# 011235813/discrete_mean_field_game

Measured on AMD Instinct MI355X. Metric: env-steps/sec for batched d-bin population rollouts, higher is better.
Workload: dtype f32 (f64 accumulate); 1 GPU; actor_critic.train(update_every="rollout") of the drop-in class (mfg_ac2.train call surface; device-side start draw every episode, one update per 15-step rollout): d=21 topics, T=15, global batch 65536 = 65536 trajectories per GPU x 1; d=21, T=15, batch_per_gpu=65536, global_batch=65536, rng=philox4x32-10, parallelism=trajectory-sharded x1, 1 all-reduce/update

## Files before the change

discrete_mean_field_game_amd/csrc/mfg_core.h:

```cpp
#pragma once
#include <hip/hip_runtime.h>
#include <stdint.h>

#include <atomic>
#include <type_traits>

#include "../../include/mfg_hip.h"
#include "mfg_device.h"

namespace mfg {

constexpr int BLOCK = 256;
constexpr int WAVES = BLOCK / WAVE;

struct CoreArgs {
  const float* pi0;
  const int32_t* start_idx;
  int64_t num_start;
  int start_draw;
  const float* pi_alpha;
  union {
    const float* P_in;
    float* pi_start_out;
  };
// ... 175 lines not shown
  T al, ad, gt;
};
template <bool SAMPLE, bool FAST>
__device__ __forceinline__ PolicyTerms<FAST> policy_terms(const PolicyElem<FAST>& e, const float4* __restrict__ htab, float th,
                                                          float v) {
  PolicyTerms<FAST> o;
  if constexpr (FAST) {
#ifdef MFG_ABL_LNY
    const float lnv = v;
#else
    const float lnv = (!SAMPLE && v == 0.0f) ? (float)(LOG_ZERO_P * INV_LN2) : (SAMPLE ? __builtin_amdgcn_logf(v) : log2_pos(v));
#endif
    o.al = e.al_f;
    o.ad = e.ad_f;
    o.gt = __builtin_fmaf(lnv, e.ad_f, -e.psi_ad);
  } else {
    const double lnv = (!SAMPLE && v == 0.0f) ? LOG_ZERO_P : log((double)v);
    o.al = e.al_d;
    o.ad = e.ad_d;
    o.gt = (-digamma_pos(e.al_d) + lnv) * e.ad_d;
  }
  return o;
}

__device__ __forceinline__ float policy_term_denormal(const PolicyElem<true>& e, float v) {
  return __builtin_fmaf(log2_pos(v), e.ad_f, -e.psi_ad);
}

template <int NE, bool TD, bool FAST, bool SEP, bool ALLVALID = false>
__device__ __forceinline__ void sample_elems_gq(const CoreArgs& a, double theta, const ThetaSplit& ts, const float* pj,
                                                const float* ej, const float* pai, const float* Fi, const uint32_t* elem,
                                                const bool* valid, uint32_t qstep, uint32_t step, uint64_t traj, float* y,
                                                typename PolicyTerms<FAST>::T* al, typename PolicyTerms<FAST>::T* ad,
                                                typename PolicyTerms<FAST>::T* gt) {
  QuadRand q;
  quad_rand(q, a.seed, elem[0], qstep, traj);
#ifndef MFG_QUAD_WIDTH
#define MFG_QUAD_WIDTH 2
#endif
  constexpr int PW = MFG_QUAD_WIDTH;
#pragma unroll
  for (int h = 0; PW * h < NE; ++h) {
    const int n2 = (NE - PW * h) >= PW ? PW : (NE - PW * h);
    PolicyElem<FAST> pe[PW];
#pragma unroll
    for (int u = 0; u < PW; ++u) {
      if (u < n2) {
        const int e = PW * h + u;
        if constexpr (SEP) policy_setup_sep<true, TD>(pe[u], a, ts, pj[e], ej[e], pai[e], Fi[e]);
        else policy_setup<true, TD, FAST>(pe[u], a, theta, ts, pj[e], pai[e]);
      }
    }
    float xn[PW], v[PW];
    bool sure[PW];
#pragma unroll
    for (int u = 0; u < PW; u += 2) {
      const int hp = (PW * h + u) >> 1;
      sure[u] = true;
      if (u + 1 < PW) sure[u + 1] = true;
#ifdef MFG_ABL_BM
      xn[u] = (q.radu[hp] - 0.5f) * 2.0f;
      if (u + 1 < PW) xn[u + 1] = (q.radu[hp] - 0.5f) * q.ang[hp];
#else
      if (u < n2) {
        const float rad = __builtin_amdgcn_sqrtf(-__builtin_amdgcn_logf(q.radu[hp]));
        xn[u] = rad * __builtin_amdgcn_cosf(q.ang[hp]);
        if (u + 1 < PW) xn[u + 1] = rad * __builtin_amdgcn_sinf(q.ang[hp]);
      }
#endif
    }
    uint64_t coldm = 0;
#pragma unroll
    for (int u = 0; u < PW; ++u) {
      if (u < n2) {
        const int e = PW * h + u;
        uint64_t cm;
        if (quad_kbits(e) == 16) v[u] = gamma_try_mask<16>(pe[u].gs, xn[u], q.kf[e], cm);
        else v[u] = gamma_try_mask<12>(pe[u].gs, xn[u], q.kf[e], cm);
        y[e] = pe[u].gs.dd * v[u];
        if constexpr (ALLVALID) coldm |= cm;
        else coldm |= cm & __builtin_amdgcn_ballot_w64(valid[e]);
      }
    }
    const bool any_cold = coldm != 0;
    if (__builtin_expect(any_cold, 0)) {
#pragma unroll
      for (int u = 0; u < PW; ++u) {
        const int e = PW * h + u;
        if (u < n2 && (ALLVALID || valid[e])) {
          const bool k16 = quad_kbits(e) == 16;
          if (k16) (void)gamma_try<16>(pe[u].gs, xn[u], q.kf[e], sure[u]);
          else (void)gamma_try<12>(pe[u].gs, xn[u], q.kf[e], sure[u]);
          if (!sure[u] || pe[u].gs.small)
            y[e] = gamma_fix(pe[u].gs, xn[u], q.kf[e], k16 ? TryConst<16>::kscale : TryConst<12>::kscale, sure[u], v[u], a.seed,
                             elem[e], step, traj);
        }
      }
    }
#pragma unroll
    for (int u = 0; u < PW; ++u) {
      if (u < n2) {
        const int e = PW * h + u;
        if (TD) {
          const PolicyTerms<FAST> t = policy_terms<true, FAST>(pe[u], a.htab, ts.th, y[e]);
          al[e] = (ALLVALID || valid[e]) ? t.al : 0;
          ad[e] = (ALLVALID || valid[e]) ? t.ad : 0;
          gt[e] = (ALLVALID || valid[e]) ? t.gt : 0;
        }
        if (!ALLVALID && !valid[e]) y[e] = 0.0f;
      }
    }
    if constexpr (TD && FAST) {
      if (__builtin_expect(any_cold, 0)) {
#pragma unroll
        for (int u = 0; u < PW; ++u) {
          const int e = PW * h + u;
          if (u < n2 && (ALLVALID || valid[e]) && y[e] < FLT_MIN_NORMAL) gt[e] = policy_term_denormal(pe[u], y[e]);
        }
      }
    }
  }
}

template <int NE, bool TD, bool FAST, bool SEP>
__device__ __forceinline__ void sample_elems_g(const CoreArgs& a, double theta, const ThetaSplit& ts, const float* pj,
                                               const float* ej, const float* pai, const float* Fi, const uint32_t* elem,
                                               const bool* valid, uint32_t step, uint64_t traj, float* y,
                                               typename PolicyTerms<FAST>::T* al, typename PolicyTerms<FAST>::T* ad,
                                               typename PolicyTerms<FAST>::T* gt) {
  sample_elems_gq<NE, TD, FAST, SEP>(a, theta, ts, pj, ej, pai, Fi, elem, valid, step, step, traj, y, al, ad, gt);
}

template <int NE, bool TD, bool FAST, bool SEP>
__device__ __forceinline__ void sample_elems(const CoreArgs& a, double theta, const ThetaSplit& ts, const float* pj,
                                             const float* ej, float pai, float Fi, uint32_t elem0, uint32_t step,
                                             uint64_t traj, float* y, float& ys, typename PolicyTerms<FAST>::T& as,
                                             typename PolicyTerms<FAST>::T& ds, typename PolicyTerms<FAST>::T& gs) {
  using TT = typename PolicyTerms<FAST>::T;
  float pa[NE], fi[NE];
  uint32_t el[NE];
  bool ok[NE];
  TT al[NE], ad[NE], gt[NE];
#pragma unroll
  for (int e = 0; e < NE; ++e) {
    pa[e] = pai;
    fi[e] = Fi;
    el[e] = elem0 + (uint32_t)e;
    ok[e] = true;
  }
  sample_elems_g<NE, TD, FAST, SEP>(a, theta, ts, pj, ej, pa, fi, el, ok, step, traj, y, al, ad, gt);
  ys = y[0];
  if (TD) {
    as = al[0];
    ds = ad[0];
    gs = gt[0];
  }
#pragma unroll
  for (int e = 1; e < NE; ++e) {
    ys += y[e];
    if (TD) {
      as += al[e];
      ds += ad[e];
      gs += gt[e];
    }
  }
}

template <bool TD, bool FAST, bool SEP>
__device__ __forceinline__ void sample_tail1(const CoreArgs& a, double theta, const ThetaSplit& ts, float pj, float ej, float pai,
                                             float Fi, uint32_t elem, uint32_t step, uint64_t traj, bool& have, float& cxn,
                                             float& ckf, float& y, typename PolicyTerms<FAST>::T& al,
                                             typename PolicyTerms<FAST>::T& ad, typename PolicyTerms<FAST>::T& gt) {
  PolicyElem<FAST> pe;
  if constexpr (SEP) policy_setup_sep<true, TD>(pe, a, ts, pj, ej, pai, Fi);
  else policy_setup<true, TD, FAST>(pe, a, theta, ts, pj, pai);
  const bool odd = (step & 1u) != 0;
  float xn, kf;
  if (odd && have) {
    xn = cxn;
    kf = ckf;
    have = false;
  } else {
    QuadRand q;
// ... 9 lines not shown
  static_assert(quad_kbits(0) == 16 && quad_kbits(1) == 16, "both integers of the first pair are 16-bit");
  uint64_t cm;
  float v = gamma_try_mask<16>(pe.gs, xn, kf, cm);
  y = pe.gs.dd * v;
  if (__builtin_expect(cm != 0, 0)) {
    bool sure = true;
    (void)gamma_try<16>(pe.gs, xn, kf, sure);
    if (!sure || pe.gs.small) y = gamma_fix(pe.gs, xn, kf, TryConst<16>::kscale, sure, v, a.seed, elem, step, traj);
  }
  if (TD) {
    const PolicyTerms<FAST> t = policy_terms<true, FAST>(pe, a.htab, ts.th, y);
    al = t.al;
    ad = t.ad;
    gt = t.gt;
    if constexpr (FAST) {
      if (__builtin_expect(cm != 0, 0) && y < FLT_MIN_NORMAL) gt = policy_term_denormal(pe, y);
    }
  }
}

__device__ __forceinline__ double value_wave(const float* pis, const double* __restrict__ w, int d, int lane) {
  const int Q = d * (d + 1) / 2;
  double acc = 0.0;
  for (int c = lane; c < d; c += WAVE) {
    const double pc = (double)pis[c];
    double col = 0.0;
    for (int i = 0; i <= c; ++i) col = fma(w[feat_idx(i, c, d)], (double)pis[i], col);
    acc = fma(pc, col + w[Q + c], acc);
  }
  acc = wave_sum(acc);
  return acc + w[Q + d];
}

#ifndef MFG_CORE_SMALL_WAVES
#define MFG_CORE_SMALL_WAVES 3
#endif
template <bool SAMPLE, bool TD, bool FAST, int D, bool SUMS = false, int STEP = 0>
#ifndef MFG_CORE_SMALL_WAVES_F64
#define MFG_CORE_SMALL_WAVES_F64 3
#endif
__device__ __forceinline__ void core_small_body(const CoreArgs& a) {
  extern __shared__ __attribute__((aligned(16))) unsigned char smem_raw[];
  MFG_STAMP0(8)
  MFG_STAMPB(0)
  const int d = D ? D : a.d;
  const int dd = d * d, dp = d | 1, T = a.T;
  const int G = WAVE / d, TB = WAVES * G;
  const int Q = d * (d + 1) / 2, F = Q + d + 1;
  const bool want_v = TD && a.w != nullptr;
  constexpr bool CIRC = SAMPLE && D > 0 && (D & 1);
  constexpr int H = (D + 1) / 2;
  const int pnw = CIRC ? 2 * d : d;
  double* wl = reinterpret_cast<double*>(smem_raw);
  double* pis64 = wl + (want_v ? ((F + 1) & ~1) : 0);
  double* red = pis64 + (SAMPLE ? 2 * TB * d : 0);
  float* tile = reinterpret_cast<float*>(red + 4 * TB * d);
  float* pis = tile + TB * d * dp;
  float* pex = pis + TB * d;
  float* pin = pex + TB * d;
  float* pal = pin + TB * 2 * d;
  double* scal = reinterpret_cast<double*>(pal + TB * d + ((TB * d) & 1));
  double* tot = scal + TB * 3;
  float* pst = reinterpret_cast<float*>(tot + TB * 8);
  const int tid = threadIdx.x, lane = tid & (WAVE - 1), wv = tid / WAVE;
  const int t = lane / d, i = lane - t * d;
  auto nblk_f = [&]() -> unsigned { return STEP == 1 ? gridDim.x - (unsigned)core_step_red_blocks(F + 3) : gridDim.x; };
  if constexpr (STEP == 1) {
    if (blockIdx.x >= nblk_f()) {
      const int64_t k = (int64_t)(blockIdx.x - nblk_f()) * WAVES + wv;
      const int64_t FO = F + 3;
      if (k >= FO) return;
      double old_val = 0.0;
      if (lane == 0) {
        if (k < F) old_val = a.w_out[k];
        else if (k == F) old_val = *a.theta;
        else if (k == F + 1 && a.pend_reward_acc) old_val = *a.pend_reward_acc;
      }
      const double gk = rows_column_sum(a.step_rows, a.step_nrows, FO, k, lane);
      if (lane == 0) {
        const double inv = 1.0 / (double)a.B;
        a.step_G[k] = gk;
        if (k < F) a.w_out[k] = updated_param(old_val, a.pend_lr_c, gk, inv);
        else if (k == F) *a.theta_out = updated_param(old_val, a.pend_lr_a, gk, inv);
        else if (k == F + 1 && a.pend_reward_acc) *a.pend_reward_acc = old_val + gk * inv;
      }
      return;
    }
  }
  float pi_first = 0.0f;
  if constexpr (STEP == 1) {
    const int64_t b0f = (int64_t)blockIdx.x * TB;
    const int tlf = wv * G + t;
    if (b0f < a.B) {
      const int64_t bf = b0f + ((t < G && b0f + tlf < a.B) ? tlf : 0);
      pi_first = a.pi0[core_src_row(a, bf) * d + i];
    }
// ... 65 lines not shown
      if (H & 1) c0 = fma(wl[(H - 1) * d + i], (double)vec[i + H - 1], c0);
      col = c0 + c1;
    } else {
      for (int k = 0, idx = i; k <= i; idx += d - k - 1, ++k) col = fma(wl[idx], (double)vec[k], col);
    }
    return (double)pi_e * (col + wl[Q + i]);
  };
  const int64_t ntiles = (a.B + TB - 1) / TB;
  for (int64_t tileid = blockIdx.x; tileid < ntiles; tileid += nblk_f()) {
    const int64_t b0 = tileid * TB;
    const int nb = (int)((a.B - b0) < TB ? (a.B - b0) : TB);
    const int tl = wv * G + t;
    const bool valid = (t < G) && (tl < nb);
    const int tlc = valid ? tl : 0;
    const int64_t b = b0 + tlc;
    double* redq = red + (size_t)tlc * 4 * d;
    float* pnv = pin + tlc * pnw;
    float pi_i = pi_first;
    {
      const int64_t tn = tileid + nblk_f();
      if (tn < ntiles) {
        const int64_t b0n = tn * TB;
        const int64_t bn = b0n + ((t < G && b0n + tl < a.B) ? tl : 0);
        pi_first = a.pi0[core_src_row(a, bn) * d + i];
      }
    }
    if (valid && a.pi_traj) a.pi_traj[b * (int64_t)(T + 1) * d + i] = pi_i;
    if constexpr (STEP == 2) {
      if (valid && a.pi_start_out) a.pi_start_out[b * d + i] = pi_i;
    }
    double v_cur = 0.0, discount = 1.0;
    bool tail_have = false;
    float tail_xn = 0.0f, tail_kf = 0.0f;
    MFG_STAMP0(10)
    for (int s = 0; s < T; ++s) {
      MFG_STAMP(0)
      tile_sync();
      float Fi = 0.0f;
      if (valid) {
        pis[tlc * d + i] = pi_i;
        if (SAMPLE && want_v && s == 0) {
          pst[tlc * pnw + i] = pi_i;
          if (CIRC) pst[tlc * pnw + d + i] = pi_i;
        }
        if (SAMPLE) pis64[2 * (tlc * d + i)] = (double)pi_i;
        if (sep) {
          pex[tlc * d + i] = exp_f64arg(theta * ((double)pi_i - SEP_CENTRE));
          Fi = exp_f64arg(-theta * ((double)pi_i + (a.shift - SEP_CENTRE)));
        }
      }
      if (!SAMPLE) {
        const int n = nb * dd;
        const float* src = a.P_in + b0 * dd;
        for (int k = tid; k < n; k += BLOCK) {
          const int row = (int)(((float)k + 0.5f) * inv_d);
          const int colj = k - row * d;
          tile[row * dp + colj] = src[k];
        }
        if (a.pi_next_in)
          for (int k = tid; k < nb * d; k += BLOCK) pin[k] = a.pi_next_in[b0 * d + k];
        if (a.pi_alpha)
          for (int k = tid; k < nb * d; k += BLOCK) pal[k] = a.pi_alpha[b0 * d + k];
      }
      tile_sync();
      MFG_STAMP(1)
      float* trow = tile + (tlc * d + i) * dp;
      const float* pv = pis + tlc * d;
      const float* pav = (!SAMPLE && a.pi_alpha) ? pal + tlc * d : pv;
      const float pai = pav[i];
      const double pid = (double)pi_i;
      double A = 0.0, D_ = 0.0, Ssum = 0.0, gacc = 0.0, racc = 0.0;
      if (valid) {
        const uint32_t step = a.first_step + (uint32_t)s;
        const uint64_t traj = a.traj_offset + (uint64_t)b;
        if (SAMPLE) {
          using TT = typename PolicyTerms<FAST>::T;
          const float* ev = pex + tlc * d;
          const uint32_t erow = (uint32_t)(i * d);
          const float pas = sep ? pai + ts.sh : pai;
          const int dq = d & ~3;
          if constexpr (D > 0 && sep) {
            typedef __attribute__((address_space(3))) const float lds_cf;
            typedef __attribute__((address_space(3))) float lds_f;
            constexpr int EOFF = WAVES * (WAVE / D) * D;
            static_assert(EOFF + 3 <= 255, "E_j must sit inside the ds_read2_b32 offset field of the pi_j base");
            lds_cf* rp = (lds_cf*)pav;
            lds_f* wp = (lds_f*)trow;
            auto quad = [&](int j, float& ys, TT& as, TT& ds, TT& gs) __attribute__((always_inline)) {
              float y[4], pjv[4], ejv[4];
#pragma unroll
              for (int e = 0; e < 4; ++e) {
                pjv[e] = rp[e];
                ejv[e] = rp[EOFF + e];
              }
              sample_elems<4, TD, FAST, sep>(a, theta, ts, pjv, ejv, pas, Fi, erow + (uint32_t)j, step, traj, y, ys, as, ds, gs);
#pragma unroll
              for (int e = 0; e < 4; ++e) wp[e] = y[e];
              rp += 4;
              wp += 4;
              asm volatile("" : "+v"(rp), "+v"(wp));
            };
#ifndef MFG_QUAD_UNROLL
#define MFG_QUAD_UNROLL 1
#endif
#pragma unroll MFG_QUAD_UNROLL
            for (int j = 0; j < dq; j += 4) {
              float ys;
              TT as, ds, gs;
              quad(j, ys, as, ds, gs);
              Ssum += (double)ys;
              if (TD) {
                A += (double)as;
                D_ += (double)ds;
                gacc += (double)gs;
              }
            }
          } else
#pragma unroll 1
          for (int j = 0; j < dq; j += 4) {
            float y[4], ys = 0.0f;
            TT as = 0, ds = 0, gs = 0;
            sample_elems<4, TD, FAST, sep>(a, theta, ts, pav + j, ev + j, pas, Fi, erow + (uint32_t)j, step, traj, y, ys,
                                           as, ds, gs);
#pragma unroll
            for (int e = 0; e < 4; ++e) trow[j + e] = y[e];
            Ssum += (double)ys;
            if (TD) {
              A += (double)as;
              D_ += (double)ds;
              gacc += (double)gs;
            }
          }
          if (dq < d) {
            float y[4], ys = 0.0f;
            TT as = 0, ds = 0, gs = 0;
            const int rem = d - dq;
            if (rem == 1)
              sample_tail1<TD, FAST, sep>(a, theta, ts, pav[dq], ev[dq], pas, Fi, erow + (uint32_t)dq, step, traj, tail_have, tail_xn,
                                          tail_kf, y[0], as, ds, gs), ys = y[0];
            else if (rem == 2)
              sample_elems<2, TD, FAST, sep>(a, theta, ts, pav + dq, ev + dq, pas, Fi, erow + (uint32_t)dq, step, traj, y,
                                             ys, as, ds, gs);
            else
              sample_elems<3, TD, FAST, sep>(a, theta, ts, pav + dq, ev + dq, pas, Fi, erow + (uint32_t)dq, step, traj, y,
                                             ys, as, ds, gs);
            for (int e = 0; e < rem; ++e) trow[dq + e] = y[e];
            Ssum += (double)ys;
            if (TD) {
              A += (double)as;
              D_ += (double)ds;
              gacc += (double)gs;
            }
          }
        } else {
          PolicyElem<FAST> pe;
#pragma unroll 2
          for (int j = 0; j < d; ++j) {
            policy_setup<SAMPLE, TD, FAST>(pe, a, theta, ts, pav[j], pai);
            const float p = trow[j];
            policy_accumulate<SAMPLE, TD, FAST>(pe, a.htab, ts.th, p, A, D_, gacc);
            racc += reward_term(a.reward_kind, pid, (double)pv[j], (double)p);
          }
        }
        MFG_STAMP(2)
        if (TD && FAST) gacc *= LN2;
        if (SAMPLE) {
          float* inv_slot = reinterpret_cast<float*>(pis64 + 2 * (tlc * d + i) + 1);
          if (FAST) {
            const float inv32 = fast_rcp_f32_of_f64(Ssum);
            if (a.P_out) {
              for (int j = 0; j < d; ++j) trow[j] *= inv32;
              *inv_slot = 1.0f;
// ... 308 lines not shown
            int k = -1;
            if (gj < D) {
              if (gi <= gj) k = feat_idx(gi, gj, D);
            } else if (gj == D) {
              if (gi <= D) k = Qc + gi;
            } else if (gj == D + 1) {
              if (gi == D) k = Fc;
            } else if (gj == D + 2) {
              if (gi == D + 1) k = Fc + 1;
            } else if (gj == D + 3) {
              if (gi == D + 1) k = Fc + 2;
            }
            const double val = tt == 0 ? c0[v] : (tt == 1 ? c1[v] : c2[v]);
            if (k >= 0) rows[wv * FO + k] = val;
          }
        }
        __syncthreads();
        for (int k = tid; k < FO; k += BLOCK) {
          double tsum = rows[k];
#pragma unroll
          for (int q = 1; q < WAVES; ++q) tsum += rows[q * FO + k];
          a.part_rows[tileid * FO + k] = tsum;
        }
        __syncthreads();
      }
    }
    MFG_STAMP0(11)
    MFG_STAMPB(1)
  }
}
template <bool SAMPLE, bool TD, bool FAST, int D, bool SUMS = false, int STEP = 0>
__global__ __launch_bounds__(BLOCK, SUMS ? 2 : (FAST ? MFG_CORE_SMALL_WAVES : MFG_CORE_SMALL_WAVES_F64)) void k_core_small(CoreArgs a) { core_small_body<SAMPLE, TD, FAST, D, SUMS, STEP>(a); }

inline size_t core_small_lds(int d, bool want_v, bool sample) {
  const int G = WAVE / d, TB = WAVES * G, dp = d | 1;
  const size_t F = (size_t)d * (d + 1) / 2 + d + 1;
  const size_t fl = (size_t)TB * d * dp + 5 * (size_t)TB * d;
  return (want_v ? ((F + 1) & ~(size_t)1) * 8 : 0) + (sample ? (size_t)2 * TB * d * 8 : 0) + (size_t)4 * TB * d * 8 + (fl + (fl & 1)) * 4 +
         (size_t)TB * 3 * 8 + (size_t)TB * 8 * 8 + (size_t)TB * 2 * d * 4;
}

#ifndef MFG_CORE_LARGE_WAVES
#define MFG_CORE_LARGE_WAVES(R) (((R) <= 2 || (R) == 4) ? 3 : 2)
#endif
#ifndef MFG_CORE_LARGE_WAVES_MIXED_SAMPLING
#define MFG_CORE_LARGE_WAVES_MIXED_SAMPLING(R) ((R) <= 2 ? 4 : ((R) <= 7 ? 3 : 2))
#endif
__host__ __device__ constexpr int large_row_batch(int R, bool td) { return R <= 2 ? 8 : (R <= 4 ? (td ? 8 : 4) : 2); }
inline size_t core_large_lds(int d, bool sample, bool fast, bool td) {
  const int R = (d + WAVE - 1) / WAVE;
  if (sample && fast) return (size_t)WAVES * ((td ? 5 : 2) * d + large_row_batch(R, td) * WAVE * R) * 4;
  return (size_t)WAVES * 4 * d * 4 + (size_t)WAVES * 3 * d * 8;
}
template <int R>
__device__ __forceinline__ void stash_store(float* p, const float* y) {
  if constexpr (R % 4 == 0) {
#pragma unroll
    for (int m = 0; m < R; m += 4) *reinterpret_cast<float4*>(p + m) = make_float4(y[m], y[m + 1], y[m + 2], y[m + 3]);
  } else if constexpr (R % 2 == 0) {
#pragma unroll
    for (int m = 0; m < R; m += 2) *reinterpret_cast<float2*>(p + m) = make_float2(y[m], y[m + 1]);
  } else {
#pragma unroll
    for (int m = 0; m < R; ++m) p[m] = y[m];
  }
}
template <int R>
__device__ __forceinline__ void stash_load(float* y, const float* p) {
  if constexpr (R % 4 == 0) {
#pragma unroll
    for (int m = 0; m < R; m += 4) {
      const float4 v = *reinterpret_cast<const float4*>(p + m);
// ... 484 lines not shown
```

discrete_mean_field_game_amd/csrc/mfg_core_small.hip:

```cpp
#include "mfg_core.h"

namespace mfg {

template <bool SAMPLE, bool TD, bool FAST, int D, bool SUMS = false, int STEP = 0>
static void go(const CoreArgs& a, int num_cus, size_t lds, hipStream_t st) {
  const int grid = core_small_grid<k_core_small<SAMPLE, TD, FAST, D, SUMS, STEP>>(a, lds, num_cus);
  hipLaunchKernelGGL((k_core_small<SAMPLE, TD, FAST, D, SUMS, STEP>), dim3(grid + (STEP == 1 ? core_step_red_blocks(a.d * (a.d + 1) / 2 + a.d + 1 + 3) : 0)), dim3(BLOCK), lds, st, a);
}

template <int D>
static void dispatch(const CoreArgs& a, bool sample, bool td, bool fast, int num_cus, size_t lds, hipStream_t st) {
  if constexpr (D > 0) {
    if (sample && td && a.step_nrows > 0) {
      if (fast) go<true, true, true, D, false, 1>(a, num_cus, lds, st);
      else go<true, true, false, D, false, 1>(a, num_cus, lds, st);
      return;
    }
    if (sample && td && a.step_nrows < 0) {
      if (fast) go<true, true, true, D, false, 2>(a, num_cus, lds, st);
      else go<true, true, false, D, false, 2>(a, num_cus, lds, st);
      return;
    }
    if (sample && td && a.part_rows) {
      if (fast) go<true, true, true, D, true>(a, num_cus, lds, st);
      else go<true, true, false, D, true>(a, num_cus, lds, st);
      return;
    }
  }
  if (fast) {
    if (sample && td) go<true, true, true, D>(a, num_cus, lds, st);
    else if (sample) go<true, false, true, D>(a, num_cus, lds, st);
    else go<false, true, true, D>(a, num_cus, lds, st);
  } else {
    if (sample && td) go<true, true, false, D>(a, num_cus, lds, st);
    else if (sample) go<true, false, false, D>(a, num_cus, lds, st);
    else go<false, true, false, D>(a, num_cus, lds, st);
  }
}

int launch_core_small(const CoreArgs& a, bool sample, bool td, bool fast, int num_cus, hipStream_t st) {
  const int d = a.d;
  if (core_row3_wanted(a, sample, td, fast, num_cus)) return launch_core_row3(a, td, num_cus, st);
  const bool want_v = td && a.w != nullptr;
  const size_t lds = core_small_lds(d, want_v, sample);
  if (d == 21) dispatch<21>(a, sample, td, fast, num_cus, lds, st);
  else if (d == 15) dispatch<15>(a, sample, td, fast, num_cus, lds, st);
  else dispatch<0>(a, sample, td, fast, num_cus, lds, st);
  return MFG_OK;
}

}
```

discrete_mean_field_game_amd/csrc/mfg_device.h:

```cpp
#pragma once
#include <hip/hip_runtime.h>
#include <stdint.h>

namespace mfg {

constexpr int WAVE = 64;
typedef double v4d_t __attribute__((ext_vector_type(4)));
constexpr float ZERO_GAMMA_REPLACEMENT = 1e-20f;
constexpr double LOG_ZERO_P = -230.25850929940458;
constexpr double LN2 = 0.6931471805599453, INV_LN2 = 1.4426950408889634;

struct u32x4 {
  uint32_t x, y, z, w;
};

__host__ __device__ __forceinline__ uint32_t xor3(uint32_t a, uint32_t b, uint32_t c) {
#if defined(__HIP_DEVICE_COMPILE__) && defined(__has_builtin)
#if __has_builtin(__builtin_amdgcn_bitop3_b32)
  return __builtin_amdgcn_bitop3_b32(a, b, c, 0x96);
#else
  return a ^ b ^ c;
#endif
#else
  return a ^ b ^ c;
#endif
}

__host__ __device__ __forceinline__ u32x4 philox4x32_10(u32x4 c, uint32_t k0, uint32_t k1) {
  constexpr uint32_t M0 = 0xD2511F53u, M1 = 0xCD9E8D57u, W0 = 0x9E3779B9u, W1 = 0xBB67AE85u;
#pragma unroll
  for (int r = 0; r < 10; ++r) {
    const uint64_t p0 = (uint64_t)M0 * c.x;
    const uint64_t p1 = (uint64_t)M1 * c.z;
    u32x4 n;
    n.x = xor3((uint32_t)(p1 >> 32), c.y, k0);
    n.y = (uint32_t)p1;
    n.z = xor3((uint32_t)(p0 >> 32), c.w, k1);
    n.w = (uint32_t)p0;
    c = n;
    k0 += W0;
    k1 += W1;
  }
  return c;
}

__device__ __forceinline__ u32x4 philox_elem(uint64_t seed, uint32_t elem, uint32_t step, uint64_t traj,
                                             uint32_t block) {
  u32x4 c;
  c.x = elem;
  c.y = step;
  c.z = (uint32_t)traj;
  c.w = ((uint32_t)(traj >> 32) & 0xFFFFu) | (block << 16);
  return philox4x32_10(c, (uint32_t)seed, (uint32_t)(seed >> 32));
}

__device__ __forceinline__ float u01(uint32_t r) { return __builtin_fmaf((float)(r >> 8), 5.9604644775390625e-8f, 2.98023223876953125e-8f); }

__device__ __forceinline__ float fast_ln(float x) { return __builtin_amdgcn_logf(x) * 0.69314718055994531f; }
__device__ __forceinline__ float fast_exp(float x) { return __builtin_amdgcn_exp2f(x * 1.44269504088896341f); }

constexpr float BM_K = 1.1774100225154747f;
constexpr float BM_K2 = 1.3862943611198906f;
struct GammaState {
  float a, dd, c;
  bool small;
};

__device__ __forceinline__ void gamma_setup(GammaState& g, float a) {
  g.a = a;
  g.small = a < 1.0f;
  const float a1 = g.small ? a + 1.0f : a;
  g.dd = a1 - (1.0f / 3.0f);
  g.c = __builtin_amdgcn_rsqf(9.0f * g.dd);
}
__device__ __forceinline__ void gamma_setup_hot(GammaState& g, float a) {
  g.a = a;
  g.small = a < 1.0f;
  g.dd = a - (1.0f / 3.0f);
  g.c = __builtin_amdgcn_rsqf((9.0f / BM_K2) * g.dd);
}
__device__ __forceinline__ void gamma_setup_hot(GammaState& g, float alpha, float scale, float scale9k) {
  g.dd = __builtin_fmaf(alpha, scale, -(1.0f / 3.0f));
  g.small = g.dd < (2.0f / 3.0f);
  g.a = g.dd + (1.0f / 3.0f);
  g.c = __builtin_amdgcn_rsqf(__builtin_fmaf(alpha, scale9k, -3.0f / BM_K2));
}

__device__ __forceinline__ bool mt_accept(const GammaState& g, float x, float u, float& v) {
  const float t = g.c * x;
  const float eps = t * (3.0f + t * (3.0f + t));
  const float x2 = x * x;
  const float tp = 1.0f + t;
  v = t < -0.5f ? tp * tp * tp : 1.0f + eps;
  bool acc = u < 1.0f - 0.0331f * x2 * x2;
  if (!acc) {
    float lme;
    if (__builtin_fabsf(eps) < 0.125f) {
      const float e2 = eps * eps;
      lme = e2 * (-0.5f + eps * (1.0f / 3.0f + eps * (-0.25f + eps * (0.2f + eps * (-1.0f / 6.0f +
            eps * (1.0f / 7.0f + eps * (-0.125f)))))));
    } else {
      lme = fast_ln(v) - eps;
    }
    acc = fast_ln(u) < 0.5f * x2 + g.dd * lme;
  }
  return acc && (t > -1.0f);
}

__device__ __forceinline__ float box_muller_radius(uint32_t r) {
  return __builtin_amdgcn_sqrtf(-1.3862943611198906f * __builtin_amdgcn_logf(u01(r)));
}

struct QuadRand {
  float radu[2];
  float ang[2];
  float kf[4];
};
__host__ __device__ constexpr int quad_kbits(int e) { return e < 2 ? 16 : 12; }

__device__ __forceinline__ void quad_rand(QuadRand& q, uint64_t seed, uint32_t elem0, uint32_t step, uint64_t traj) {
#ifdef MFG_ABL_PHILOX
  u32x4 r;
  r.x = (elem0 + step) * 2654435761u ^ (uint32_t)traj;
  r.y = r.x * 2246822519u + 12345u;
  r.z = r.y ^ (r.x >> 7);
  r.w = r.z * 3266489917u;
#else
  const u32x4 r = philox_elem(seed, elem0, step, traj, 0);
#endif
  q.ang[0] = __builtin_fmaf((float)(r.z >> 16), 1.52587890625e-5f, 7.62939453125e-6f);
  q.ang[1] = __builtin_fmaf((float)(r.z & 0xFFFFu), 1.52587890625e-5f, 7.62939453125e-6f);
  q.radu[0] = __builtin_fmaf((float)(r.x >> 12), 9.5367431640625e-7f, 4.76837158203125e-7f);
  q.radu[1] = __builtin_fmaf((float)(r.y >> 12), 9.5367431640625e-7f, 4.76837158203125e-7f);
  q.kf[0] = (float)(r.w >> 16);
  q.kf[1] = (float)(r.w & 0xFFFFu);
  q.kf[2] = (float)(r.x & 0xFFFu);
  q.kf[3] = (float)(r.y & 0xFFFu);
}

__device__ __forceinline__ float gamma_exact_path(const GammaState& g, float x, float kf, float kscale, uint64_t seed,
                                                  uint32_t elem, uint32_t step, uint64_t traj) {
  float v = 1.0f;
  {
    const u32x4 r = philox_elem(seed, elem, step, traj, 1);
    const float u = (kf + u01(r.x)) * kscale;
    if (mt_accept(g, x, u, v)) return v;
  }
  for (uint32_t block = 2; block < 64; ++block) {
    const u32x4 r = philox_elem(seed, elem, step, traj, block);
    const float xn = box_muller_radius(r.x) * __builtin_amdgcn_cosf(u01(r.y));
    if (mt_accept(g, xn, u01(r.z), v)) return v;
  }
  return 1.0f;
}

template <int KB>
struct TryConst {
  static constexpr float slope = KB == 16 ? -12451.84f * 1.3862944f : -778.24f * 1.3862944f;
  static constexpr float top = KB == 16 ? 65532.7f : 4094.85f;
  static constexpr float kscale = KB == 16 ? 1.52587890625e-5f : 2.44140625e-4f;
};
template <int KB = 12>
__device__ __forceinline__ float gamma_try(const GammaState& g, float x, float kf, bool& sure) {
#ifdef MFG_ABL_TRY
  sure = true;
  return 1.0f + 3.0f * g.c * x;
#endif
  const float t = g.c * x;
  const float q = x * t;
  const float thr = __builtin_fmaf(q * q, TryConst<KB>::slope, TryConst<KB>::top);
// ... 159 lines not shown
struct ThetaSplit {
  float th, tl, sh, c0;
  float thn;
};
__device__ __forceinline__ ThetaSplit theta_split(double theta, double shift) {
  ThetaSplit t;
  t.th = (float)theta;
  t.tl = (float)(theta - (double)t.th);
  t.sh = (float)shift;
  t.c0 = t.th * (float)(shift - (double)t.sh);
  t.thn = t.th * 16.0f;
  return t;
}
__device__ __forceinline__ void theta_times_x(const ThetaSplit& t, float pj, float pi, float& x, float& zh, float& zl) {
  x = (pj - pi) - t.sh;
  zh = t.th * x;
  zl = __builtin_fmaf(t.th, x, -zh) + __builtin_fmaf(t.tl, x, -t.c0);
}

constexpr float HTAB_ZMIN = -24.0f;
constexpr float HTAB_ZMAX = 88.0f;
constexpr int HTAB_PER_UNIT = 16;
constexpr int HTAB_N = (88 + 24) * HTAB_PER_UNIT;

__device__ __forceinline__ float htab_eval(const float4* __restrict__ tab, float x, float thn) {
#ifdef MFG_ABL_HTAB
  return x * thn * 0.1f;
#endif
  static_assert(HTAB_PER_UNIT == 16, "ThetaSplit::thn assumes 16 intervals per unit of z");
  float t = __builtin_fmaf(x, thn, -HTAB_ZMIN * (float)HTAB_PER_UNIT);
  t = __builtin_amdgcn_fmed3f(t, 0.0f, (float)HTAB_N - 0.001f);
  const unsigned k = (unsigned)t;
  const float f = __builtin_amdgcn_fractf(t);
  const float4 c = tab[k];
  return __builtin_fmaf(__builtin_fmaf(__builtin_fmaf(c.w, f, c.z), f, c.y), f, c.x);
}

template <int CTRL, int ROW_MASK>
__device__ __forceinline__ double dpp_mov_f64(double v) {
  int lo = __double2loint(v), hi = __double2hiint(v);
  if (ROW_MASK == 0xF) {
    lo = __builtin_amdgcn_update_dpp(0, lo, CTRL, 0xF, 0xF, true);
    hi = __builtin_amdgcn_update_dpp(0, hi, CTRL, 0xF, 0xF, true);
  } else {
    lo = __builtin_amdgcn_update_dpp(0, lo, CTRL, ROW_MASK, 0xF, false);
    hi = __builtin_amdgcn_update_dpp(0, hi, CTRL, ROW_MASK, 0xF, false);
  }
  return __hiloint2double(hi, lo);
}

__device__ __forceinline__ double wave_sum_dpp(double v) {
  v += dpp_mov_f64<0xB1, 0xF>(v);
  v += dpp_mov_f64<0x4E, 0xF>(v);
  v += dpp_mov_f64<0x141, 0xF>(v);
  v += dpp_mov_f64<0x140, 0xF>(v);
  v += dpp_mov_f64<0x142, 0xA>(v);
  v += dpp_mov_f64<0x143, 0xC>(v);
  const int lo = __builtin_amdgcn_readlane(__double2loint(v), 63);
  const int hi = __builtin_amdgcn_readlane(__double2hiint(v), 63);
  return __hiloint2double(hi, lo);
}


__device__ __forceinline__ void wave_sum3_dpp(double& a, double& b, double& c) {
#define MFG_SUM3_STEP(CTRL, MASK)                 \
  {                                               \
    const double ta = dpp_mov_f64<CTRL, MASK>(a); \
// ... 165 lines not shown
```

discrete_mean_field_game_amd/csrc/mfg_evaluate_pop.hip:

```cpp
#include "mfg_core.h"
#include "mfg_evaluate_pop.h"

namespace mfg {

template <bool FAST, int D>
__global__ __launch_bounds__(BLOCK, FAST ? MFG_CORE_SMALL_WAVES : 2) void k_eval_rollout_pop(CoreArgs a, PopArgs p) {
  const int k = blockIdx.y;
  const int d = D ? D : a.d;
  const int TB = WAVES * (WAVE / d);
  int32_t* idx = p.idx + p.s_idx * k;
  for (int64_t b0 = (int64_t)blockIdx.x * TB; b0 < a.B; b0 += (int64_t)gridDim.x * TB) {
    const int64_t b = b0 + threadIdx.x;
    if (threadIdx.x < TB && b < a.B) idx[b] = (int32_t)((b % p.N) * p.L);
  }
  __threadfence();
  __syncthreads();
  CoreArgs c = pop_core_args<false, 0>(a, p, k);
  c.start_idx = idx;
  core_small_body<true, false, FAST, D, false, 0>(c);
}

template <bool FAST, int D>
static void go_eval(const CoreArgs& a, const PopArgs& p, int num_cus, size_t lds, hipStream_t st) {
  const int grid = core_small_grid<k_eval_rollout_pop<FAST, D>>(a, lds, num_cus);
  hipLaunchKernelGGL((k_eval_rollout_pop<FAST, D>), dim3((unsigned)grid, (unsigned)p.K), dim3(BLOCK), lds, st, a, p);
}

int launch_eval_rollout_pop(const CoreArgs& a, const PopArgs& p, bool fast, int num_cus, hipStream_t st) {
  const int d = a.d;
  if (d > WAVE) return MFG_EUNSUPPORTED;
  const size_t lds = core_small_lds(d, false, true);
  if (d == 21) {
    if (fast) go_eval<true, 21>(a, p, num_cus, lds, st);
    else go_eval<false, 21>(a, p, num_cus, lds, st);
  } else if (d == 15) {
    if (fast) go_eval<true, 15>(a, p, num_cus, lds, st);
    else go_eval<false, 15>(a, p, num_cus, lds, st);
  } else {
    if (fast) go_eval<true, 0>(a, p, num_cus, lds, st);
    else go_eval<false, 0>(a, p, num_cus, lds, st);
  }
  return MFG_OK;
}

__global__ __launch_bounds__(BLOCK) void k_eval_metrics_pop(const float* __restrict__ gen_all, const float* __restrict__ emp32,
                                                            const double* __restrict__ emp64, int64_t N, int L, int d, int64_t NR,
                                                            double* __restrict__ per_traj_all, double* __restrict__ metrics) {
  __shared__ double part[WAVES][4];
  __shared__ double mean_s[4];
  const int k = blockIdx.x;
  const int lane = threadIdx.x & (WAVE - 1), wv = threadIdx.x / WAVE;
  const float* gen = gen_all + (int64_t)k * NR * L * d;
  double* per_traj = per_traj_all + (int64_t)k * NR * 4;
  const bool on = lane < d;
  double s[4] = {0.0, 0.0, 0.0, 0.0};
  for (int64_t j = wv; j < NR; j += WAVES) {
    const int64_t n = j % N;
    double l1_sum = 0.0, jsd_sum = 0.0, l1 = 0.0, jsd = 0.0;
    for (int l = 0; l < L; ++l) {
      const int64_t eo = (n * L + l) * d + lane;
      double a = 1.0, c = 1.0, e1 = 0.0;
      if (on) {
        const float g = gen[(j * L + l) * d + lane];
        e1 = fabs(emp64[eo] - (double)g);
// ... 64 lines not shown
```

discrete_mean_field_game_amd/csrc/mfg_population.hip:

```cpp
#include "mfg_core.h"
#define MFG_GRAD_BODIES_ONLY
#include "mfg_grad.h"
#include "mfg_population.h"

namespace mfg {

template <bool FAST, int D, bool SUMS, int STEP>
__global__ __launch_bounds__(BLOCK, SUMS ? 2 : (FAST ? MFG_CORE_SMALL_WAVES : MFG_CORE_SMALL_WAVES_F64)) void k_core_pop(CoreArgs a,
                                                                                                                   PopArgs p) {
  core_small_body<true, true, FAST, D, SUMS, STEP>(pop_core_args<SUMS, STEP>(a, p, blockIdx.y));
}

template <bool FAST, int D, bool SUMS, int STEP>
static void go_pop(const CoreArgs& a, const PopArgs& p, int num_cus, size_t lds, hipStream_t st) {
  const int grid = core_small_grid<k_core_pop<FAST, D, SUMS, STEP>>(a, lds, num_cus) +
                   (STEP == 1 ? core_step_red_blocks(a.d * (a.d + 1) / 2 + a.d + 1 + 3) : 0);
  hipLaunchKernelGGL((k_core_pop<FAST, D, SUMS, STEP>), dim3((unsigned)grid, (unsigned)p.K), dim3(BLOCK), lds, st, a, p);
}

template <int D>
static void dispatch_pop(const CoreArgs& a, const PopArgs& p, bool fast, int num_cus, size_t lds, hipStream_t st) {
  if constexpr (D > 0) {
    if (a.step_nrows > 0) {
      if (fast) go_pop<true, D, false, 1>(a, p, num_cus, lds, st);
      else go_pop<false, D, false, 1>(a, p, num_cus, lds, st);
      return;
    }
    if (a.step_nrows < 0) {
      if (fast) go_pop<true, D, false, 2>(a, p, num_cus, lds, st);
      else go_pop<false, D, false, 2>(a, p, num_cus, lds, st);
      return;
    }
    if (a.part_rows) {
      if (fast) go_pop<true, D, true, 0>(a, p, num_cus, lds, st);
      else go_pop<false, D, true, 0>(a, p, num_cus, lds, st);
      return;
    }
  }
  if (fast) go_pop<true, D, false, 0>(a, p, num_cus, lds, st);
  else go_pop<false, D, false, 0>(a, p, num_cus, lds, st);
}

int launch_core_pop(const CoreArgs& a, const PopArgs& p, bool fast, int num_cus, hipStream_t st) {
  const int d = a.d;
  if (d > WAVE) return MFG_EUNSUPPORTED;
  const size_t lds = core_small_lds(d, a.w != nullptr, true);
  if (d == 21) dispatch_pop<21>(a, p, fast, num_cus, lds, st);
  else if (d == 15) dispatch_pop<15>(a, p, fast, num_cus, lds, st);
  else if (!a.part_rows && a.step_nrows == 0) dispatch_pop<0>(a, p, fast, num_cus, lds, st);
  else return MFG_EUNSUPPORTED;
  return MFG_OK;
}

__global__ void k_draw_start_pop(const float* __restrict__ mat, int64_t num_start, int64_t B, int d, uint32_t step,
                                 uint64_t traj_offset, float* __restrict__ out, PopArgs p) {
  const int k = blockIdx.y;
  draw_start_body(mat, num_start, B, d, p.seed[k], step, traj_offset, nullptr, out + p.s_state * k);
}

void launch_draw_start_pop(int grid, const float* mat, int64_t num_start, int64_t B, int d, uint32_t step, uint64_t traj_offset,
                           float* out, const PopArgs& p, hipStream_t st) {
  hipLaunchKernelGGL(k_draw_start_pop, dim3((unsigned)grid, (unsigned)p.K), dim3(256), 0, st, mat, num_start, B, d, step,
                     traj_offset, out, p);
}

__device__ __forceinline__ void pop_rebase_grad(GradArgs& a, const PopArgs& p, int k) {
  a.pi += p.s_gpi * k;
  a.delta += p.s_n * k;
  a.g += p.s_n * k;
  a.reward = pop_at(a.reward, p.s_n, k);
  a.partial = pop_bytes(a.partial, p.s_ws, k);
  a.counter = pop_bytes(a.counter, p.s_ws, k);
  a.G = pop_at(a.G, p.F + 3, k);
  a.w = pop_at(a.w, p.F, k);
  a.theta = pop_at(a.theta, 1, k);
  a.reward_acc = pop_at(a.reward_acc, p.s_acc, k);
  a.lr_c = p.lr_c[k] * p.sc;
  a.lr_a = p.lr_a[k] * p.sa;
}
// ... 79 lines not shown
```

Baseline: 1.057 billion env-steps/s.

## Precompute step-invariant Philox rounds per trajectory and cache them in LDS

The counter-based Philox generator is split into a part that depends only on element and trajectory and a part that depends on step. The first one and a half rounds for each element quad are computed once per trajectory before the step loop and stored in LDS. Each step then finishes the remaining rounds from that cached state. This removes repeated Philox work from the hot sampling loop at the cost of extra LDS per block, which may reduce occupancy. A small table-lookup addressing tweak is also included.

Result: no change. 1.052 billion env-steps/s (-0.5%).

```diff
diff --git a/discrete_mean_field_game_amd/csrc/mfg_core.h b/discrete_mean_field_game_amd/csrc/mfg_core.h
--- a/discrete_mean_field_game_amd/csrc/mfg_core.h
+++ b/discrete_mean_field_game_amd/csrc/mfg_core.h
@@ -231,9 +231,10 @@
                                                 const float* ej, const float* pai, const float* Fi, const uint32_t* elem,
                                                 const bool* valid, uint32_t qstep, uint32_t step, uint64_t traj, float* y,
                                                 typename PolicyTerms<FAST>::T* al, typename PolicyTerms<FAST>::T* ad,
-                                                typename PolicyTerms<FAST>::T* gt) {
+                                                typename PolicyTerms<FAST>::T* gt, const u32x4* blk = nullptr, uint32_t ecold = 0) {
   QuadRand q;
-  quad_rand(q, a.seed, elem[0], qstep, traj);
+  if (blk) quad_fields(q, *blk);
+  else quad_rand(q, a.seed, elem[0], qstep, traj);
 #ifndef MFG_QUAD_WIDTH
 #define MFG_QUAD_WIDTH 2
 #endif
@@ -283,6 +284,8 @@
     }
     const bool any_cold = coldm != 0;
     if (__builtin_expect(any_cold, 0)) {
+      uint32_t ec = ecold;
+      asm volatile("" : "+s"(ec));
 #pragma unroll
       for (int u = 0; u < PW; ++u) {
         const int e = PW * h + u;
@@ -292,7 +295,7 @@
           else (void)gamma_try<12>(pe[u].gs, xn[u], q.kf[e], sure[u]);
           if (!sure[u] || pe[u].gs.small)
             y[e] = gamma_fix(pe[u].gs, xn[u], q.kf[e], k16 ? TryConst<16>::kscale : TryConst<12>::kscale, sure[u], v[u], a.seed,
-                             elem[e], step, traj);
+                             elem[e] + ec, step, traj);
         }
       }
     }
@@ -326,15 +329,16 @@
                                                const float* ej, const float* pai, const float* Fi, const uint32_t* elem,
                                                const bool* valid, uint32_t step, uint64_t traj, float* y,
                                                typename PolicyTerms<FAST>::T* al, typename PolicyTerms<FAST>::T* ad,
-                                               typename PolicyTerms<FAST>::T* gt) {
-  sample_elems_gq<NE, TD, FAST, SEP>(a, theta, ts, pj, ej, pai, Fi, elem, valid, step, step, traj, y, al, ad, gt);
+                                               typename PolicyTerms<FAST>::T* gt, const u32x4* blk = nullptr, uint32_t ecold = 0) {
+  sample_elems_gq<NE, TD, FAST, SEP>(a, theta, ts, pj, ej, pai, Fi, elem, valid, step, step, traj, y, al, ad, gt, blk, ecold);
 }
 
 template <int NE, bool TD, bool FAST, bool SEP>
 __device__ __forceinline__ void sample_elems(const CoreArgs& a, double theta, const ThetaSplit& ts, const float* pj,
                                              const float* ej, float pai, float Fi, uint32_t elem0, uint32_t step,
                                              uint64_t traj, float* y, float& ys, typename PolicyTerms<FAST>::T& as,
-                                             typename PolicyTerms<FAST>::T& ds, typename PolicyTerms<FAST>::T& gs) {
+                                             typename PolicyTerms<FAST>::T& ds, typename PolicyTerms<FAST>::T& gs,
+                                             const u32x4* blk = nullptr, uint32_t ecold = 0) {
   using TT = typename PolicyTerms<FAST>::T;
   float pa[NE], fi[NE];
   uint32_t el[NE];
@@ -347,7 +351,7 @@
     el[e] = elem0 + (uint32_t)e;
     ok[e] = true;
   }
-  sample_elems_g<NE, TD, FAST, SEP>(a, theta, ts, pj, ej, pa, fi, el, ok, step, traj, y, al, ad, gt);
+  sample_elems_g<NE, TD, FAST, SEP>(a, theta, ts, pj, ej, pa, fi, el, ok, step, traj, y, al, ad, gt, blk, ecold);
   ys = y[0];
   if (TD) {
     as = al[0];
@@ -423,6 +427,7 @@
   return acc + w[Q + d];
 }
 
+__host__ __device__ constexpr bool core_small_quad_fixed(int d, bool sample, bool fast) { return sample && fast && (d == 21 || d == 15); }
 #ifndef MFG_CORE_SMALL_WAVES
 #define MFG_CORE_SMALL_WAVES 3
 #endif
@@ -453,6 +458,7 @@
   double* scal = reinterpret_cast<double*>(pal + TB * d + ((TB * d) & 1));
   double* tot = scal + TB * 3;
   float* pst = reinterpret_cast<float*>(tot + TB * 8);
+  uint64_t* qfix = reinterpret_cast<uint64_t*>(pst + TB * 2 * d);
   const int tid = threadIdx.x, lane = tid & (WAVE - 1), wv = tid / WAVE;
   const int t = lane / d, i = lane - t * d;
   auto nblk_f = [&]() -> unsigned { return STEP == 1 ? gridDim.x - (unsigned)core_step_red_blocks(F + 3) : gridDim.x; };
@@ -584,6 +590,15 @@
     double v_cur = 0.0, discount = 1.0;
     bool tail_have = false;
     float tail_xn = 0.0f, tail_kf = 0.0f;
+    if constexpr (core_small_quad_fixed(D, SAMPLE, FAST)) {
+      if (valid) {
+        uint32_t e0 = (uint32_t)(i * d);
+        asm volatile("" : "+v"(e0));
+#pragma unroll
+        for (int q = 0; q < D / 4; ++q)
+          qfix[q * BLOCK + tid] = philox_quad_fixed(a.seed, e0 + (uint32_t)(4 * q), a.traj_offset + (uint64_t)b);
+      }
+    }
     MFG_STAMP0(10)
     for (int s = 0; s < T; ++s) {
       MFG_STAMP(0)
@@ -636,8 +651,15 @@
             typedef __attribute__((address_space(3))) float lds_f;
             constexpr int EOFF = WAVES * (WAVE / D) * D;
             static_assert(EOFF + 3 <= 255, "E_j must sit inside the ds_read2_b32 offset field of the pi_j base");
+            static_assert(core_small_quad_fixed(D, SAMPLE, FAST), "this loop reads qfix: core_small_lds must have made room for it");
             lds_cf* rp = (lds_cf*)pav;
             lds_f* wp = (lds_f*)trow;
+#ifndef MFG_ABL_PHILOX
+            typedef __attribute__((address_space(3))) const uint64_t lds_cu64;
+            lds_cu64* qp = (lds_cu64*)(qfix + tid);
+            const uint64_t qstp = philox_quad_step(a.seed, step, traj);
+            uint32_t qnw = PHILOX_M0 * erow;
+#endif
             auto quad = [&](int j, float& ys, TT& as, TT& ds, TT& gs) __attribute__((always_inline)) {
               float y[4], pjv[4], ejv[4];
 #pragma unroll
@@ -645,7 +667,15 @@
                 pjv[e] = rp[e];
                 ejv[e] = rp[EOFF + e];
               }
+#ifndef MFG_ABL_PHILOX
+              const u32x4 blk = philox_quad_finish(a.seed, *qp, qstp, qnw);
+              sample_elems<4, TD, FAST, sep>(a, theta, ts, pjv, ejv, pas, Fi, erow, step, traj, y, ys, as, ds, gs, &blk, (uint32_t)j);
+              qnw += 4u * PHILOX_M0;
+              qp += BLOCK;
+              asm volatile("" : "+v"(qp));
+#else
               sample_elems<4, TD, FAST, sep>(a, theta, ts, pjv, ejv, pas, Fi, erow + (uint32_t)j, step, traj, y, ys, as, ds, gs);
+#endif
 #pragma unroll
               for (int e = 0; e < 4; ++e) wp[e] = y[e];
               rp += 4;
@@ -687,9 +717,12 @@
             float y[4], ys = 0.0f;
             TT as = 0, ds = 0, gs = 0;
             const int rem = d - dq;
-            if (rem == 1)
-              sample_tail1<TD, FAST, sep>(a, theta, ts, pav[dq], ev[dq], pas, Fi, erow + (uint32_t)dq, step, traj, tail_have, tail_xn,
-                                          tail_kf, y[0], as, ds, gs), ys = y[0];
+            if (rem == 1) {
+              uint32_t et = erow + (uint32_t)dq;
+              if constexpr (core_small_quad_fixed(D, SAMPLE, FAST)) asm volatile("" : "+v"(et));
+              sample_tail1<TD, FAST, sep>(a, theta, ts, pav[dq], ev[dq], pas, Fi, et, step, traj, tail_have, tail_xn, tail_kf, y[0], as, ds,
+                                          gs), ys = y[0];
+            }
             else if (rem == 2)
               sample_elems<2, TD, FAST, sep>(a, theta, ts, pav + dq, ev + dq, pas, Fi, erow + (uint32_t)dq, step, traj, y,
                                              ys, as, ds, gs);
@@ -1064,12 +1097,13 @@
 template <bool SAMPLE, bool TD, bool FAST, int D, bool SUMS = false, int STEP = 0>
 __global__ __launch_bounds__(BLOCK, SUMS ? 2 : (FAST ? MFG_CORE_SMALL_WAVES : MFG_CORE_SMALL_WAVES_F64)) void k_core_small(CoreArgs a) { core_small_body<SAMPLE, TD, FAST, D, SUMS, STEP>(a); }
 
-inline size_t core_small_lds(int d, bool want_v, bool sample) {
+inline size_t core_small_lds(int d, bool want_v, bool sample, bool fast) {
   const int G = WAVE / d, TB = WAVES * G, dp = d | 1;
   const size_t F = (size_t)d * (d + 1) / 2 + d + 1;
   const size_t fl = (size_t)TB * d * dp + 5 * (size_t)TB * d;
   return (want_v ? ((F + 1) & ~(size_t)1) * 8 : 0) + (sample ? (size_t)2 * TB * d * 8 : 0) + (size_t)4 * TB * d * 8 + (fl + (fl & 1)) * 4 +
-         (size_t)TB * 3 * 8 + (size_t)TB * 8 * 8 + (size_t)TB * 2 * d * 4;
+         (size_t)TB * 3 * 8 + (size_t)TB * 8 * 8 + (size_t)TB * 2 * d * 4 +
+         (core_small_quad_fixed(d, sample, fast) ? (size_t)(d / 4) * BLOCK * 8 : 0);
 }
 
 #ifndef MFG_CORE_LARGE_WAVES
diff --git a/discrete_mean_field_game_amd/csrc/mfg_core_small.hip b/discrete_mean_field_game_amd/csrc/mfg_core_small.hip
--- a/discrete_mean_field_game_amd/csrc/mfg_core_small.hip
+++ b/discrete_mean_field_game_amd/csrc/mfg_core_small.hip
@@ -42,7 +42,7 @@
   const int d = a.d;
   if (core_row3_wanted(a, sample, td, fast, num_cus)) return launch_core_row3(a, td, num_cus, st);
   const bool want_v = td && a.w != nullptr;
-  const size_t lds = core_small_lds(d, want_v, sample);
+  const size_t lds = core_small_lds(d, want_v, sample, fast);
   if (d == 21) dispatch<21>(a, sample, td, fast, num_cus, lds, st);
   else if (d == 15) dispatch<15>(a, sample, td, fast, num_cus, lds, st);
   else dispatch<0>(a, sample, td, fast, num_cus, lds, st);
diff --git a/discrete_mean_field_game_amd/csrc/mfg_device.h b/discrete_mean_field_game_amd/csrc/mfg_device.h
--- a/discrete_mean_field_game_amd/csrc/mfg_device.h
+++ b/discrete_mean_field_game_amd/csrc/mfg_device.h
@@ -52,6 +52,41 @@
   c.z = (uint32_t)traj;
   c.w = ((uint32_t)(traj >> 32) & 0xFFFFu) | (block << 16);
   return philox4x32_10(c, (uint32_t)seed, (uint32_t)(seed >> 32));
+}
+
+constexpr uint32_t PHILOX_M0 = 0xD2511F53u, PHILOX_M1 = 0xCD9E8D57u, PHILOX_W0 = 0x9E3779B9u, PHILOX_W1 = 0xBB67AE85u;
+__device__ __forceinline__ uint64_t philox_quad_fixed(uint64_t seed, uint32_t elem0, uint64_t traj) {
+  const uint32_t k0 = (uint32_t)seed, k1 = (uint32_t)(seed >> 32);
+  const uint32_t c3 = (uint32_t)(traj >> 32) & 0xFFFFu;
+  const uint32_t z1 = xor3((uint32_t)(((uint64_t)PHILOX_M0 * elem0) >> 32), c3, k1);
+  const uint64_t p1 = (uint64_t)PHILOX_M1 * z1;
+  return (uint64_t)xor3((uint32_t)(p1 >> 32), PHILOX_M1 * (uint32_t)traj, k0 + PHILOX_W0) | ((uint64_t)(uint32_t)p1 << 32);
+}
+__device__ __forceinline__ uint64_t philox_quad_step(uint64_t seed, uint32_t step, uint64_t traj) {
+  const uint32_t x1 = xor3((uint32_t)(((uint64_t)PHILOX_M1 * (uint32_t)traj) >> 32), step, (uint32_t)seed);
+  return (uint64_t)PHILOX_M0 * x1;
+}
+__device__ __forceinline__ u32x4 philox_quad_finish(uint64_t seed, uint64_t fixed, uint64_t stp, uint32_t nw) {
+  uint32_t k0 = (uint32_t)seed + PHILOX_W0, k1 = (uint32_t)(seed >> 32) + PHILOX_W1;
+  u32x4 c;
+  c.x = (uint32_t)fixed;
+  c.y = (uint32_t)(fixed >> 32);
+  c.z = xor3((uint32_t)(stp >> 32), nw, k1);
+  c.w = (uint32_t)stp;
+#pragma unroll
+  for (int r = 2; r < 10; ++r) {
+    k0 += PHILOX_W0;
+    k1 += PHILOX_W1;
+    const uint64_t p0 = (uint64_t)PHILOX_M0 * c.x;
+    const uint64_t p1 = (uint64_t)PHILOX_M1 * c.z;
+    u32x4 n;
+    n.x = xor3((uint32_t)(p1 >> 32), c.y, k0);
+    n.y = (uint32_t)p1;
+    n.z = xor3((uint32_t)(p0 >> 32), c.w, k1);
+    n.w = (uint32_t)p0;
+    c = n;
+  }
+  return c;
 }
 
 __device__ __forceinline__ float u01(uint32_t r) { return __builtin_fmaf((float)(r >> 8), 5.9604644775390625e-8f, 2.98023223876953125e-8f); }
@@ -118,6 +153,16 @@
 };
 __host__ __device__ constexpr int quad_kbits(int e) { return e < 2 ? 16 : 12; }
 
+__device__ __forceinline__ void quad_fields(QuadRand& q, const u32x4& r) {
+  q.ang[0] = __builtin_fmaf((float)(r.z >> 16), 1.52587890625e-5f, 7.62939453125e-6f);
+  q.ang[1] = __builtin_fmaf((float)(r.z & 0xFFFFu), 1.52587890625e-5f, 7.62939453125e-6f);
+  q.radu[0] = __builtin_fmaf((float)(r.x >> 12), 9.5367431640625e-7f, 4.76837158203125e-7f);
+  q.radu[1] = __builtin_fmaf((float)(r.y >> 12), 9.5367431640625e-7f, 4.76837158203125e-7f);
+  q.kf[0] = (float)(r.w >> 16);
+  q.kf[1] = (float)(r.w & 0xFFFFu);
+  q.kf[2] = (float)(r.x & 0xFFFu);
+  q.kf[3] = (float)(r.y & 0xFFFu);
+}
 __device__ __forceinline__ void quad_rand(QuadRand& q, uint64_t seed, uint32_t elem0, uint32_t step, uint64_t traj) {
 #ifdef MFG_ABL_PHILOX
   u32x4 r;
@@ -128,14 +173,7 @@
 #else
   const u32x4 r = philox_elem(seed, elem0, step, traj, 0);
 #endif
-  q.ang[0] = __builtin_fmaf((float)(r.z >> 16), 1.52587890625e-5f, 7.62939453125e-6f);
-  q.ang[1] = __builtin_fmaf((float)(r.z & 0xFFFFu), 1.52587890625e-5f, 7.62939453125e-6f);
-  q.radu[0] = __builtin_fmaf((float)(r.x >> 12), 9.5367431640625e-7f, 4.76837158203125e-7f);
-  q.radu[1] = __builtin_fmaf((float)(r.y >> 12), 9.5367431640625e-7f, 4.76837158203125e-7f);
-  q.kf[0] = (float)(r.w >> 16);
-  q.kf[1] = (float)(r.w & 0xFFFFu);
-  q.kf[2] = (float)(r.x & 0xFFFu);
-  q.kf[3] = (float)(r.y & 0xFFFu);
+  quad_fields(q, r);
 }
 
 __device__ __forceinline__ float gamma_exact_path(const GammaState& g, float x, float kf, float kscale, uint64_t seed,
@@ -361,7 +399,7 @@
   t = __builtin_amdgcn_fmed3f(t, 0.0f, (float)HTAB_N - 0.001f);
   const unsigned k = (unsigned)t;
   const float f = __builtin_amdgcn_fractf(t);
-  const float4 c = tab[k];
+  const float4 c = *reinterpret_cast<const float4*>(reinterpret_cast<const char*>(tab) + (k << 4));
   return __builtin_fmaf(__builtin_fmaf(__builtin_fmaf(c.w, f, c.z), f, c.y), f, c.x);
 }
 
diff --git a/discrete_mean_field_game_amd/csrc/mfg_evaluate_pop.hip b/discrete_mean_field_game_amd/csrc/mfg_evaluate_pop.hip
--- a/discrete_mean_field_game_amd/csrc/mfg_evaluate_pop.hip
+++ b/discrete_mean_field_game_amd/csrc/mfg_evaluate_pop.hip
@@ -29,7 +29,7 @@
 int launch_eval_rollout_pop(const CoreArgs& a, const PopArgs& p, bool fast, int num_cus, hipStream_t st) {
   const int d = a.d;
   if (d > WAVE) return MFG_EUNSUPPORTED;
-  const size_t lds = core_small_lds(d, false, true);
+  const size_t lds = core_small_lds(d, false, true, fast);
   if (d == 21) {
     if (fast) go_eval<true, 21>(a, p, num_cus, lds, st);
     else go_eval<false, 21>(a, p, num_cus, lds, st);
diff --git a/discrete_mean_field_game_amd/csrc/mfg_population.hip b/discrete_mean_field_game_amd/csrc/mfg_population.hip
--- a/discrete_mean_field_game_amd/csrc/mfg_population.hip
+++ b/discrete_mean_field_game_amd/csrc/mfg_population.hip
@@ -44,7 +44,7 @@
 int launch_core_pop(const CoreArgs& a, const PopArgs& p, bool fast, int num_cus, hipStream_t st) {
   const int d = a.d;
   if (d > WAVE) return MFG_EUNSUPPORTED;
-  const size_t lds = core_small_lds(d, a.w != nullptr, true);
+  const size_t lds = core_small_lds(d, a.w != nullptr, true, fast);
   if (d == 21) dispatch_pop<21>(a, p, fast, num_cus, lds, st);
   else if (d == 15) dispatch_pop<15>(a, p, fast, num_cus, lds, st);
   else if (!a.part_rows && a.step_nrows == 0) dispatch_pop<0>(a, p, fast, num_cus, lds, st);
```
